# yassouali/pytorch-segmentation

Measured on NVIDIA H100. Metric: images/sec DeepLabV3+/ResNet101 513x513 train step (fwd+CE+bwd+SGD), higher is better.
Workload: dtype bf16

## Files before the change

### pytorch-segmentation_b200/csrc/seg_conv_tc.cu

```cuda
#include <cuda.h>
#include <mutex>
#include <stdlib.h>
#include "seg_common.cuh"
#include "seg_ptx.cuh"
#include "seg_sync.cuh"

namespace seg {
namespace tc {

using namespace ptx;

constexpr int BM = 128;
constexpr int BK = 64;
constexpr int A_BYTES = BM * 128;
constexpr int KIND_KK = 0, KIND_KM = 1;
constexpr int NTHREADS = 384;
constexpr int NCONS = 256;
constexpr int MAXT = 49;

constexpr int BAR_CONSUMERS = 1;
constexpr int BAR_ORDER = 2;
constexpr int BAR_WG = 4;

struct TcParams {
  CUtensorMap mapA;
  CUtensorMap mapB;
  int M;
  int Ncols;
  int taps;
  int kchunks;
  int stride;
  int lower_h, lower_w;
  int PQ, Q;
  int x_im2col;
  int brows_per_tap;
  short tap_wt[MAXT];
  short tap_oh[MAXT];
  short tap_ow[MAXT];
  void* out;
  long long ldo;
  int out_dtype;
  float beta;
  const float* bias;
  double* stats;
  int stat_rows;
  unsigned* stat_ticket;
  SyncDesc sync;
  int out_strided, out_H, out_W, osy, osx, opy, opx;
  int n_tiles, tiles;
  int kblocks_total, kblocks_per_split;
  float* dw;
  int dw_K, dw_C;
  float* ws;
};

__device__ __forceinline__ void row_to_coords(int m, int PQ, int Q, int stride, int lower_h, int lower_w, int& n, int& h,
                                              int& w) {
  n = m / PQ;
  int rem = m - n * PQ;
  int pp = rem / Q;
  int qq = rem - pp * Q;
  h = lower_h + pp * stride;
  w = lower_w + qq * stride;
}

template <int BN, int TA, int TB>
__device__ __forceinline__ void wgmma_tile(float* acc, uint64_t adesc, uint64_t bdesc, uint32_t accumulate) {
  if constexpr (BN == 64) wgmma_m64n64k16<TA, TB>(acc, adesc, bdesc, accumulate);
  else if constexpr (BN == 128) wgmma_m64n128k16<TA, TB>(acc, adesc, bdesc, accumulate);
  else wgmma_m64n256k16<TA, TB>(acc, adesc, bdesc, accumulate);
}

template <int BN, int KIND>
__device__ __forceinline__ void load_kblock(const TcParams& p, uint32_t a_dst, uint32_t bar, int kc, int wtap, uint16_t oh,
                                            uint16_t ow, int n_img, int h0, int w0, int m0, int n0) {
  const uint32_t b_dst = a_dst + A_BYTES;
  if (p.x_im2col)
    tma_load_im2col_4d(a_dst, &p.mapA, bar, kc * BK, w0, h0, n_img, ow, oh);
  else
    tma_load_2d(a_dst, &p.mapA, bar, kc * BK, m0);
  if (KIND == KIND_KK) {
    tma_load_2d(b_dst, &p.mapB, bar, kc * BK, wtap * p.brows_per_tap + n0);
  } else {
#pragma unroll
    for (int j = 0; j < BN / 64; ++j)
      tma_load_2d(b_dst + j * 8192, &p.mapB, bar, n0 + j * 64, wtap * p.brows_per_tap + kc * BK);
  }
}

template <int BN>
__device__ __forceinline__ void stage_acc(const float* acc, const float* acc1, uint8_t* stage, int rbase, int warp, int lane,
                                          const float* bias, bool out_f32) {
  const int esize = out_f32 ? 4 : 2;
  const int CPR = BN * esize / 16;
  const int swz = (CPR >= 32 ? 31 : CPR - 1);
  const int r0 = rbase + warp * 16 + (lane >> 2);
#pragma unroll
  for (int j = 0; j < BN / 8; ++j) {
    const int col = j * 8 + 2 * (lane & 3);
    float b0 = 0.f, b1 = 0.f;
    if (bias) {
      b0 = bias[col];
      b1 = bias[col + 1];
    }
#pragma unroll
    for (int h = 0; h < 4; ++h) {
      if (h >= 2 && !acc1) break;
      const float* a = h < 2 ? acc : acc1;
      const int r = r0 + 8 * (h & 1) + 32 * (h & 2);
      const float x0 = a[4 * j + 2 * (h & 1)] + b0, x1 = a[4 * j + 2 * (h & 1) + 1] + b1;
      const int byte = col * esize;
      uint8_t* dst = stage + (size_t)r * (BN * esize) + ((((byte >> 4) ^ (r & swz))) << 4) + (byte & 15);
      if (out_f32)
        *reinterpret_cast<float2*>(dst) = make_float2(x0, x1);
      else
        *reinterpret_cast<__nv_bfloat162*>(dst) = __floats2bfloat162_rn(x0, x1);
    }
  }
}


template <int BN, int ESIZE>
__device__ __forceinline__ void store_tile(const TcParams& p, const uint8_t* stage, int tid, int m0, int n0, int ncols_tile) {
  constexpr int CPR = BN * ESIZE / 16;
  constexpr int swz = (CPR >= 32 ? 31 : CPR - 1);
  constexpr int RSTEP = 128 / CPR;
  constexpr int NCH = BM / RSTEP;
  constexpr int BATCH = 8;
  static_assert(128 % CPR == 0 && NCH % BATCH == 0, "chunk walk of the staged tile");
  const int c16 = tid % CPR;
  const int nchunks = (ncols_tile * ESIZE + 15) >> 4;
  if (c16 >= nchunks) return;
  const bool vec_ok = ((p.ldo * ESIZE) & 15) == 0 && ((reinterpret_cast<uintptr_t>(p.out) + (size_t)n0 * ESIZE) & 15) == 0;
  const int first_col = (c16 << 4) / ESIZE;
  const bool full = first_col + 16 / ESIZE <= ncols_tile;
  auto row_dst = [&](int tr) {
    const int grow = m0 + tr;
    long long pixel = grow;
    if (p.out_strided) {
      const int n = grow / p.PQ;
      const int rem = grow - n * p.PQ;
      const int i = rem / p.Q, jj = rem - i * p.Q;
      pixel = ((long long)n * p.out_H + (i * p.osy + p.opy)) * p.out_W + (jj * p.osx + p.opx);
    }
    return reinterpret_cast<uint8_t*>(p.out) + ((size_t)pixel * p.ldo + n0) * ESIZE + ((size_t)c16 << 4);
  };
  auto row_src = [&](int tr) { return stage + (size_t)tr * (BN * ESIZE) + ((c16 ^ (tr & swz)) << 4); };
  if (ESIZE == 2 && vec_ok && full && p.beta != 0.f) {
    for (int b = 0; b < NCH; b += BATCH) {
      uint8_t* dst[BATCH];
      uint4 old[BATCH];
#pragma unroll
      for (int u = 0; u < BATCH; ++u) {
        const int tr = tid / CPR + (b + u) * RSTEP;
        dst[u] = m0 + tr < p.M ? row_dst(tr) : nullptr;
        old[u] = dst[u] ? *reinterpret_cast<const uint4*>(dst[u]) : make_uint4(0u, 0u, 0u, 0u);
      }
#pragma unroll
      for (int u = 0; u < BATCH; ++u) {
        if (!dst[u]) continue;
        float a[8], o[8];
        unpack8(*reinterpret_cast<const bf16x8*>(row_src(tid / CPR + (b + u) * RSTEP)), a);
        unpack8(*reinterpret_cast<const bf16x8*>(&old[u]), o);
#pragma unroll
        for (int k = 0; k < 8; ++k) a[k] += p.beta * o[k];
        *reinterpret_cast<bf16x8*>(dst[u]) = pack8(a);
      }
    }
    return;
  }
  for (int tr = tid / CPR; tr < BM; tr += RSTEP) {
    if (m0 + tr >= p.M) break;
    const uint8_t* src = row_src(tr);
    uint8_t* dst = row_dst(tr);
    if (ESIZE == 2 && vec_ok && full) {
      *reinterpret_cast<bf16x8*>(dst) = *reinterpret_cast<const bf16x8*>(src);
    } else if (ESIZE == 2) {
      float a[8];
      unpack8(*reinterpret_cast<const bf16x8*>(src), a);
      __nv_bfloat16* d = reinterpret_cast<__nv_bfloat16*>(dst);
      for (int k = 0; k < 8; ++k)
        if (first_col + k < ncols_tile) {
          float o = a[k];
          if (p.beta != 0.f) o += p.beta * bf2f(d[k]);
          d[k] = f2bf(o);
        }
    } else {
      const float4 val = *reinterpret_cast<const float4*>(src);
      const float a[4] = {val.x, val.y, val.z, val.w};
      float* d = reinterpret_cast<float*>(dst);
      if (vec_ok && full && p.beta == 0.f) {
        *reinterpret_cast<float4*>(d) = val;
      } else {
        for (int k = 0; k < 4; ++k)
          if (first_col + k < ncols_tile) d[k] = (p.beta != 0.f) ? a[k] + p.beta * d[k] : a[k];
      }
    }
  }
}

template <int BN>
struct PPCfg {
  static_assert(BN == 64 || BN == 128, "ping-pong tile width");
  static constexpr int B_BYTES = BN * 128;
  static constexpr int STAGE_BYTES = A_BYTES + B_BYTES;
  static constexpr int STAGES = BN == 64 ? 6 : 4;
  static constexpr int RING = STAGES * STAGE_BYTES;
  static constexpr int STG_BYTES = BM * 256;
  static constexpr int MAXG = BM / 32;
  static constexpr int STAT_BYTES = MAXG * 2 * BN * 4 + BN * 4;
  static constexpr int SMEM = RING + 2 * (STG_BYTES + STAT_BYTES) + 1024  + 256 ;
  static_assert(16 * STAGES + 8 <= 256, "barrier area");
  static_assert(SMEM <= 227 * 1024, "shared memory per block");
};

template <int BN, int KIND>
__global__ void __launch_bounds__(NTHREADS, 1) conv_gemm_pp(const __grid_constant__ TcParams p) {
  using C = PPCfg<BN>;
  constexpr int STAGES = C::STAGES;
  extern __shared__ uint8_t smem_raw[];
  const uint32_t raw_addr = smem_u32(smem_raw);
  const uint32_t smem0 = (raw_addr + 1023u) & ~1023u;
  uint8_t* smem_gen = smem_raw + (smem0 - raw_addr);
  const uint32_t bar0 = smem0 + C::RING + 2 * (C::STG_BYTES + C::STAT_BYTES);
  auto full_bar = [&](int s) { return bar0 + 8u * s; };
  auto empty_bar = [&](int s) { return bar0 + 8u * (STAGES + s); };
  volatile int* flag_sm = reinterpret_cast<volatile int*>(smem_gen + (bar0 - smem0) + 16 * STAGES);

  const int num_iters = p.taps * p.kchunks;
  const int grid = gridDim.x;
  const int ntiles = (p.tiles - (int)blockIdx.x + grid - 1) / grid;

  if (threadIdx.x == 0) {
    prefetch_tmap(&p.mapA);
    prefetch_tmap(&p.mapB);
    for (int s = 0; s < STAGES; ++s) {
      mbar_init(full_bar(s), 1);
      mbar_init(empty_bar(s), 4);
    }
    fence_mbar_init();
  }
  __syncthreads();
  pdl_wait();

  if (threadIdx.x < 128) {
    setmaxnreg_dec<40>();
    if (threadIdx.x == 0 && num_iters > 0) {
      int it = 0;
      for (int j = 0; j < ntiles; ++j) {
        const int t = blockIdx.x + j * grid;
        const int m0 = (t / p.n_tiles) * BM, n0 = (t % p.n_tiles) * BN;
        int n_img = 0, h0 = 0, w0 = 0;
        if (p.x_im2col) row_to_coords(m0, p.PQ, p.Q, p.stride, p.lower_h, p.lower_w, n_img, h0, w0);
        for (int tap = 0; tap < p.taps; ++tap) {
          const int wtap = p.tap_wt[tap];
          const uint16_t oh = (uint16_t)p.tap_oh[tap], ow = (uint16_t)p.tap_ow[tap];
          for (int kc = 0; kc < p.kchunks; ++kc, ++it) {
            const int st = it % STAGES;
            mbar_wait_nocall(empty_bar(st), ((it / STAGES) & 1) ^ 1u);
            mbar_arrive_expect_tx(full_bar(st), C::STAGE_BYTES);
            load_kblock<BN, KIND>(p, smem0 + st * C::STAGE_BYTES, full_bar(st), kc, wtap, oh, ow, n_img, h0, w0, m0, n0);
          }
        }
      }
    }
    return;
  }

  setmaxnreg_inc<232>();
  const int cw = (threadIdx.x - 128) >> 7;
  const int tid = threadIdx.x & 127;
  const int warp = tid >> 5, lane = tid & 31;
  uint8_t* stage = smem_gen + C::RING + cw * C::STG_BYTES;
  float* stat_sm = reinterpret_cast<float*>(smem_gen + C::RING + 2 * C::STG_BYTES + cw * C::STAT_BYTES);
  float* bias_sm = stat_sm + C::MAXG * 2 * BN;
  const bool out_f32 = p.out_dtype != SEG_DT_BF16;
  const int esize = out_f32 ? 4 : 2;
  const int CPR = BN * esize / 16;
  const int swz = (CPR >= 32 ? 31 : CPR - 1);
  auto wg_sync = [&] { named_sync(BAR_WG + cw, 128); };

  for (int j = cw; j < ntiles; j += 2) {
    const int t = blockIdx.x + j * grid;
    const int m0 = (t / p.n_tiles) * BM, n0 = (t % p.n_tiles) * BN;
    float acc0[BN / 2], acc1[BN / 2];
#pragma unroll
    for (int i = 0; i < BN / 2; ++i) acc0[i] = acc1[i] = 0.f;

    if (j > 0) named_sync(BAR_ORDER + cw, NCONS);
    {
      constexpr int TB = (KIND == KIND_KK) ? 0 : 1;
      const int it0 = j * num_iters;
      for (int i = 0; i < num_iters; ++i) {
        const int it = it0 + i;
        const int st = it % STAGES;
        mbar_wait_nocall(full_bar(st), (it / STAGES) & 1);
        const uint32_t a_addr = smem0 + st * C::STAGE_BYTES;
        const uint32_t b_addr = a_addr + A_BYTES;
        const uint64_t adesc0 = make_smem_desc_sw128(a_addr, 16, 1024);
        const uint64_t adesc1 = make_smem_desc_sw128(a_addr + 8192, 16, 1024);
        const uint64_t bdesc0 = make_smem_desc_sw128(b_addr, TB ? 8192 : 16, 1024);
        wgmma_fence();
#pragma unroll
        for (int k = 0; k < BK / 16; ++k) {
          const uint64_t bdesc = bdesc0 + (uint64_t)(TB ? (k * 2048 >> 4) : (k * 32 >> 4));
          wgmma_tile<BN, 0, TB>(acc0, adesc0 + (uint64_t)(k * 32 >> 4), bdesc, 1u);
          wgmma_tile<BN, 0, TB>(acc1, adesc1 + (uint64_t)(k * 32 >> 4), bdesc, 1u);
        }
        wgmma_commit();
        wgmma_wait<1>();
        __syncwarp();
        if (i > 0 && lane == 0) mbar_arrive(empty_bar((it - 1) % STAGES));
      }
      if (j + 1 < ntiles) named_arrive(BAR_ORDER + (cw ^ 1), NCONS);
      wgmma_wait<0>();
      __syncwarp();
      if (num_iters > 0 && lane == 0) mbar_arrive(empty_bar((it0 + num_iters - 1) % STAGES));
    }

    const int ncols_tile = min(BN, p.Ncols - n0);
    if (p.bias && tid < BN) bias_sm[tid] = tid < ncols_tile ? __ldg(p.bias + n0 + tid) : 0.f;
    wg_sync();
    stage_acc<BN>(acc0, acc1, stage, 0, warp, lane, p.bias ? bias_sm : nullptr, out_f32);
    wg_sync();

    const int ngroups = BM / p.stat_rows;
    if (p.stats) {
      const int parts = min(128 / BN, ngroups);
      const int rpp = BM / parts;
      const int c = tid % BN, part = tid / BN;
      const int rvalid = min(BM, p.M - m0);
      if (part < parts) {
        const int byte = c * esize;
        int g = part * rpp / p.stat_rows;
        auto load = [&](int r) {
          const uint8_t* src = stage + (size_t)r * (BN * esize) + ((((byte >> 4) ^ (r & swz))) << 4) + (byte & 15);
          return out_f32 ? *reinterpret_cast<const float*>(src) : bf2f(*reinterpret_cast<const __nv_bfloat16*>(src));
        };
        for (int rg = part * rpp; rg < (part + 1) * rpp; rg += p.stat_rows, ++g) {
          float s1 = 0.f, s2 = 0.f;
          const int rend = min(rg + p.stat_rows, rvalid);
          int r = rg;
          for (; r + 8 <= rend; r += 8) {
            float x[8];
#pragma unroll
            for (int u = 0; u < 8; ++u) x[u] = load(r + u);
#pragma unroll
            for (int u = 0; u < 8; ++u) {
              s1 += x[u];
              s2 = fmaf(x[u], x[u], s2);
            }
          }
          for (; r < rend; ++r) {
            const float x = load(r);
            s1 += x;
            s2 = fmaf(x, x, s2);
          }
          stat_sm[(g * 2 + 0) * BN + c] = s1;
          stat_sm[(g * 2 + 1) * BN + c] = s2;
        }
      }
    }

    if (out_f32)
      store_tile<BN, 4>(p, stage, tid, m0, n0, ncols_tile);
    else
      store_tile<BN, 2>(p, stage, tid, m0, n0, ncols_tile);
    if (j == ntiles - 1 && tid == 0) pdl_trigger();

    if (p.stats) {
      wg_sync();
      if (tid < ncols_tile) {
        float a = 0.f, b = 0.f;
        for (int g = 0; g < ngroups; ++g) {
          a += stat_sm[(g * 2 + 0) * BN + tid];
          b += stat_sm[(g * 2 + 1) * BN + tid];
        }
        atomicAdd(p.stats + n0 + tid, (double)a);
        atomicAdd(p.stats + p.Ncols + n0 + tid, (double)b);
      }
    }
  }

  if (p.stats && p.sync.world > 0)
    sync_push_when_last<false>(p.sync, p.stats, 2 * p.Ncols, p.stat_ticket, gridDim.x, threadIdx.x - 128, NCONS,
                               [] { named_sync(BAR_CONSUMERS, NCONS); }, flag_sm);
}


template <int BN>
struct Cfg {
  static constexpr int B_BYTES = BN * 128;
  static constexpr int STAGE_BYTES = A_BYTES + B_BYTES;
  static constexpr int STAGES = BN == 64 ? 6 : (BN == 128 ? 5 : 4);
  static constexpr int SMEM = STAGES * STAGE_BYTES + 1024  + 256 ;
  static_assert(STAGES * STAGE_BYTES >= BM * BN * 4, "staging tile must fit in the pipeline ring");
  static_assert(SMEM <= 227 * 1024, "shared memory per block");
};

template <int BN>
__global__ void __launch_bounds__(NTHREADS, 1) conv_gemm_wgrad(const __grid_constant__ TcParams p) {
  using C = Cfg<BN>;
  constexpr int STAGES = C::STAGES;
  extern __shared__ uint8_t smem_raw[];
  const uint32_t raw_addr = smem_u32(smem_raw);
  const uint32_t smem0 = (raw_addr + 1023u) & ~1023u;
  uint8_t* smem_gen = smem_raw + (smem0 - raw_addr);
  const uint32_t bar0 = smem0 + STAGES * C::STAGE_BYTES;
  auto full_bar = [&](int s) { return bar0 + 8u * s; };
  auto empty_bar = [&](int s) { return bar0 + 8u * (STAGES + s); };

  const int m0 = blockIdx.x * BM;
  const int n0 = blockIdx.y * BN;

  const int tap_mm = blockIdx.z % p.taps;
  const int split = blockIdx.z / p.taps;
  const int kb_begin = split * p.kblocks_per_split;
  const int kb_end = min(kb_begin + p.kblocks_per_split, p.kblocks_total);
  const int num_iters = max(kb_end - kb_begin, 0);

  if (threadIdx.x == 0) {
    prefetch_tmap(&p.mapA);
    prefetch_tmap(&p.mapB);
    for (int s = 0; s < STAGES; ++s) {
      mbar_init(full_bar(s), 1);
      mbar_init(empty_bar(s), 8);
    }
    fence_mbar_init();
  }
  __syncthreads();
  pdl_wait();

  if (threadIdx.x < 128) {
    if (threadIdx.x == 0 && num_iters > 0) {
      const uint16_t oh = (uint16_t)p.tap_oh[tap_mm], ow = (uint16_t)p.tap_ow[tap_mm];
      int it = 0;
      for (int kb = kb_begin; kb < kb_end; ++kb, ++it) {
        const int st = it % STAGES;
        const uint32_t ph = (it / STAGES) & 1;
        mbar_wait_nocall(empty_bar(st), ph ^ 1u);
        const uint32_t a_dst = smem0 + st * C::STAGE_BYTES;
        const uint32_t b_dst = a_dst + A_BYTES;
        const int pix0 = kb * BK;
        mbar_arrive_expect_tx(full_bar(st), C::STAGE_BYTES);
        tma_load_2d(a_dst, &p.mapA, full_bar(st), m0, pix0);
        tma_load_2d(a_dst + 8192, &p.mapA, full_bar(st), m0 + 64, pix0);
        if (p.x_im2col) {
          int n_img, h0, w0;
          row_to_coords(pix0, p.PQ, p.Q, p.stride, p.lower_h, p.lower_w, n_img, h0, w0);
#pragma unroll
          for (int j = 0; j < BN / 64; ++j)
            tma_load_im2col_4d(b_dst + j * 8192, &p.mapB, full_bar(st), n0 + j * 64, w0, h0, n_img, ow, oh);
        } else {
#pragma unroll
          for (int j = 0; j < BN / 64; ++j) tma_load_2d(b_dst + j * 8192, &p.mapB, full_bar(st), n0 + j * 64, pix0);
        }
      }
    }
    return;
  }

  if (num_iters == 0) return;
  const int ctid = threadIdx.x - 128;
  const int cw = ctid >> 7;
  const int warp = (ctid >> 5) & 3, lane = ctid & 31;
  float acc[BN / 2];
#pragma unroll
  for (int i = 0; i < BN / 2; ++i) acc[i] = 0.f;
  for (int it = 0; it < num_iters; ++it) {
    const int st = it % STAGES;
    mbar_wait_nocall(full_bar(st), (it / STAGES) & 1);
    const uint32_t a_addr = smem0 + st * C::STAGE_BYTES + cw * 8192;
    const uint32_t b_addr = smem0 + st * C::STAGE_BYTES + A_BYTES;
    const uint64_t adesc0 = make_smem_desc_sw128(a_addr, 8192, 1024);
    const uint64_t bdesc0 = make_smem_desc_sw128(b_addr, 8192, 1024);
    wgmma_fence();
#pragma unroll
    for (int k = 0; k < BK / 16; ++k)
      wgmma_tile<BN, 1, 1>(acc, adesc0 + (uint64_t)(k * 2048 >> 4), bdesc0 + (uint64_t)(k * 2048 >> 4), 1u);
    wgmma_commit();
    wgmma_wait<1>();
    __syncwarp();
    if (it > 0 && lane == 0) mbar_arrive(empty_bar((it - 1) % STAGES));
  }
  wgmma_wait<0>();
  named_sync(BAR_CONSUMERS, NCONS);

  uint8_t* stage = smem_gen;
  const int ncols_tile = min(BN, p.Ncols - n0);
  stage_acc<BN>(acc, nullptr, stage, cw * 64, warp, lane, nullptr, true);
  named_sync(BAR_CONSUMERS, NCONS);

  const int CPR = BN * 4 / 16;
  const int swz = (CPR >= 32 ? 31 : CPR - 1);
  float* base = p.ws ? p.ws + (size_t)split * p.taps * p.dw_K * p.dw_C : p.dw;
  for (int idx = ctid; idx < BM * CPR; idx += NCONS) {
    const int tr = idx / CPR, c16 = idx - tr * CPR;
    const int row = m0 + tr, col0 = c16 * 4;
    if (row >= p.M || col0 >= ncols_tile) continue;
    const float4 v = *reinterpret_cast<const float4*>(stage + (size_t)tr * (BN * 4) + ((c16 ^ (tr & swz)) << 4));
    float* dst = base + ((size_t)tap_mm * p.dw_K + row) * p.dw_C + n0 + col0;
    const bool vec = col0 + 4 <= ncols_tile && ((reinterpret_cast<uintptr_t>(dst) & 15) == 0);
    const float a[4] = {v.x, v.y, v.z, v.w};
    if (p.ws) {
      if (vec)
        *reinterpret_cast<float4*>(dst) = v;
      else
        for (int i = 0; i < 4; ++i)
          if (col0 + i < ncols_tile) dst[i] = a[i];
    } else if (vec) {
      asm volatile("red.global.add.v4.f32 [%0], {%1, %2, %3, %4};" ::"l"(dst), "f"(v.x), "f"(v.y), "f"(v.z), "f"(v.w)
                   : "memory");
    } else {
      for (int i = 0; i < 4; ++i)
        if (col0 + i < ncols_tile) atomicAdd(dst + i, a[i]);
    }
  }
}

typedef CUresult (*EncodeTiledFn)(CUtensorMap*, CUtensorMapDataType, cuuint32_t, void*, const cuuint64_t*,
                                  const cuuint64_t*, const cuuint32_t*, const cuuint32_t*, CUtensorMapInterleave,
                                  CUtensorMapSwizzle, CUtensorMapL2promotion, CUtensorMapFloatOOBfill);
typedef CUresult (*EncodeIm2colFn)(CUtensorMap*, CUtensorMapDataType, cuuint32_t, void*, const cuuint64_t*,
                                   const cuuint64_t*, const int*, const int*, cuuint32_t, cuuint32_t,
                                   const cuuint32_t*, CUtensorMapInterleave, CUtensorMapSwizzle,
                                   CUtensorMapL2promotion, CUtensorMapFloatOOBfill);
static EncodeTiledFn g_encode_tiled = nullptr;
static EncodeIm2colFn g_encode_im2col = nullptr;
static int g_driver_version = 0;

static int resolve_driver() {
  static std::once_flag once;
  static int status = 0;
  std::call_once(once, [] {
    void* f1 = nullptr;
    void* f2 = nullptr;
    cudaDriverEntryPointQueryResult q;
    if (cudaGetDriverEntryPoint("cuTensorMapEncodeTiled", &f1, cudaEnableDefault, &q) != cudaSuccess || !f1) status = 1;
    if (cudaGetDriverEntryPoint("cuTensorMapEncodeIm2col", &f2, cudaEnableDefault, &q) != cudaSuccess || !f2) status = 1;
    g_encode_tiled = (EncodeTiledFn)f1;
    g_encode_im2col = (EncodeIm2colFn)f2;
    cudaDriverGetVersion(&g_driver_version);
  });
  if (status) set_error("cannot resolve cuTensorMapEncode* driver entry points");
  return status;
}

static int make_map_2d(CUtensorMap* m, const void* ptr, int64_t rows, int64_t cols, int64_t ld, int box_rows) {
  if (resolve_driver()) return 1;
  SEG_REQUIRE((reinterpret_cast<uintptr_t>(ptr) & 15) == 0, "TMA: base pointer not 16-byte aligned");
  SEG_REQUIRE(ld % 8 == 0, "TMA: row pitch %lld not a multiple of 8 elements", (long long)ld);
  cuuint64_t dims[2] = {(cuuint64_t)cols, (cuuint64_t)rows};
  cuuint64_t strides[1] = {(cuuint64_t)ld * 2};
  cuuint32_t box[2] = {64, (cuuint32_t)box_rows};
  cuuint32_t es[2] = {1, 1};
  CUresult r = g_encode_tiled(m, CU_TENSOR_MAP_DATA_TYPE_BFLOAT16, 2, const_cast<void*>(ptr), dims, strides, box, es,
                              CU_TENSOR_MAP_INTERLEAVE_NONE, CU_TENSOR_MAP_SWIZZLE_128B,
                              CU_TENSOR_MAP_L2_PROMOTION_L2_256B, CU_TENSOR_MAP_FLOAT_OOB_FILL_NONE);
  SEG_REQUIRE(r == CUDA_SUCCESS, "cuTensorMapEncodeTiled failed (%d) rows=%lld cols=%lld ld=%lld box_rows=%d", (int)r,
              (long long)rows, (long long)cols, (long long)ld, box_rows);
  return 0;
}

static int make_map_im2col(CUtensorMap* m, const void* ptr, int N, int H, int W, int C, int64_t ld, int lower_w,
                           int lower_h, int upper_w, int upper_h, int stride, int pixels) {
  if (resolve_driver()) return 1;
  SEG_REQUIRE((reinterpret_cast<uintptr_t>(ptr) & 15) == 0, "TMA: base pointer not 16-byte aligned");
  SEG_REQUIRE(ld % 8 == 0, "TMA: channel pitch %lld not a multiple of 8", (long long)ld);
  SEG_REQUIRE(lower_w >= -128 && upper_w >= -128 && lower_w <= 127 && upper_w <= 127 && lower_h >= -128 &&
                  upper_h >= -128 && lower_h <= 127 && upper_h <= 127,
              "im2col corner out of range");
  cuuint64_t dims[4] = {(cuuint64_t)C, (cuuint64_t)W, (cuuint64_t)H, (cuuint64_t)N};
  cuuint64_t strides[3] = {(cuuint64_t)ld * 2, (cuuint64_t)W * ld * 2, (cuuint64_t)H * W * ld * 2};
  int lo[2] = {lower_w, lower_h};
  int up[2] = {upper_w, upper_h};
  cuuint32_t es[4] = {1, (cuuint32_t)stride, (cuuint32_t)stride, 1};
  CUresult r = g_encode_im2col(m, CU_TENSOR_MAP_DATA_TYPE_BFLOAT16, 4, const_cast<void*>(ptr), dims, strides, lo, up,
                               64, (cuuint32_t)pixels, es, CU_TENSOR_MAP_INTERLEAVE_NONE, CU_TENSOR_MAP_SWIZZLE_128B,
                               CU_TENSOR_MAP_L2_PROMOTION_L2_256B, CU_TENSOR_MAP_FLOAT_OOB_FILL_NONE);
  SEG_REQUIRE(r == CUDA_SUCCESS,
              "cuTensorMapEncodeIm2col failed (%d) N=%d H=%d W=%d C=%d ld=%lld lo=(%d,%d) up=(%d,%d) s=%d", (int)r, N, H,
              W, C, (long long)ld, lower_w, lower_h, upper_w, upper_h, stride);
  if (g_driver_version <= 13010) {
    const uint64_t bytes = (uint64_t)N * H * W * ld * 2;
    if (bytes < 131072) reinterpret_cast<uint64_t*>(m)[1] &= ~(1ull << 21);
  }
  return 0;
}

template <int BN, int KIND>
static int launch_pp(TcParams& p, cudaStream_t stream) {
  static bool attr_set = false;
  auto kfn = conv_gemm_pp<BN, KIND>;
  if (!attr_set) {
    cudaError_t e = cudaFuncSetAttribute(kfn, cudaFuncAttributeMaxDynamicSharedMemorySize, PPCfg<BN>::SMEM);
    SEG_REQUIRE(e == cudaSuccess, "cudaFuncSetAttribute(smem=%d): %s", PPCfg<BN>::SMEM, cudaGetErrorString(e));
    attr_set = true;
  }
  const int n_tiles = ceil_div(p.Ncols, BN);
  const int64_t tiles = ceil_div64(p.M, BM) * n_tiles;
  SEG_REQUIRE(tiles < (1ll << 31), "too many output tiles");
  p.n_tiles = n_tiles;
  p.tiles = (int)tiles;
  const dim3 grid((unsigned)std::min<int64_t>(tiles, num_sms()));
  launch_pdl(kfn, grid, dim3(NTHREADS), (size_t)PPCfg<BN>::SMEM, stream, p);
  return check_launch("conv_gemm_pp");
}

template <int KIND>
static int launch_pp_bn(int bn, TcParams& p, cudaStream_t stream) {
  switch (bn) {
    case 64: return launch_pp<64, KIND>(p, stream);
    case 128: return launch_pp<128, KIND>(p, stream);
  }
  set_error("bad BN %d", bn);
  return 1;
}

template <int BN>
static int launch_wgrad(const TcParams& p, dim3 grid, cudaStream_t stream) {
  static bool attr_set = false;
  auto kfn = conv_gemm_wgrad<BN>;
  if (!attr_set) {
    cudaError_t e = cudaFuncSetAttribute(kfn, cudaFuncAttributeMaxDynamicSharedMemorySize, Cfg<BN>::SMEM);
    SEG_REQUIRE(e == cudaSuccess, "cudaFuncSetAttribute(smem=%d): %s", Cfg<BN>::SMEM, cudaGetErrorString(e));
    attr_set = true;
  }
  launch_pdl(kfn, grid, dim3(NTHREADS), (size_t)Cfg<BN>::SMEM, stream, p);
  return check_launch("conv_gemm_wgrad");
}

static int launch_wgrad_bn(int bn, const TcParams& p, dim3 grid, cudaStream_t stream) {
  switch (bn) {
    case 64: return launch_wgrad<64>(p, grid, stream);
    case 128: return launch_wgrad<128>(p, grid, stream);
    case 256: return launch_wgrad<256>(p, grid, stream);
  }
  set_error("bad BN %d", bn);
  return 1;
}

static int pick_bn(int ncols, bool out_f32) { return (ncols <= 64 || out_f32) ? 64 : 128; }

static int stat_rows_for(int ncols) {
  if (ncols <= 64) return 32;
  if (ncols < 256) return 64;
  return ceil_div(ncols, 256) * 256 - ncols < 128 ? 128 : 64;
}

bool supported(const seg_conv_desc* d) {
  if (d->C % 8 != 0 || d->ldx % 8 != 0) return false;
  if (d->R != d->S) return false;
  if (d->R * d->S > MAXT) return false;
  if (d->pad > 127 || d->dil * (d->R - 1) - d->pad > 127 || d->dil * (d->R - 1) - d->pad < -127) return false;
  if (d->stride > 8) return false;
  return true;
}

static bool is_pointwise(const seg_conv_desc* d) { return d->R == 1 && d->S == 1 && d->stride == 1 && d->pad == 0; }

int conv_fwd(const seg_conv_desc* d, const void* x, const void* w, void* y, int y_dtype, const float* bias, float beta,
             double* stats, unsigned* stat_ticket, const SyncDesc* sync, cudaStream_t stream) {
  SEG_REQUIRE(supported(d), "wgmma conv fwd: unsupported shape (C=%d ldx=%d R=%d pad=%d dil=%d)", d->C, d->ldx, d->R,
              d->pad, d->dil);
  TcParams p;
  memset(&p, 0, sizeof(p));
  const int64_t M = (int64_t)d->N * d->P * d->Q;
  SEG_REQUIRE(M < (1ll << 31), "M too large");
  p.M = (int)M;
  p.Ncols = d->K;
  p.taps = d->R * d->S;
  for (int t = 0; t < p.taps; ++t) {
    p.tap_wt[t] = (short)t;
    p.tap_oh[t] = (short)((t / d->S) * d->dil);
    p.tap_ow[t] = (short)((t % d->S) * d->dil);
  }
  p.kchunks = ceil_div(d->C, BK);
  p.stride = d->stride;
  p.lower_h = p.lower_w = -d->pad;
  p.PQ = d->P * d->Q;
  p.Q = d->Q;
  p.brows_per_tap = d->K;
  p.out = y;
  p.ldo = d->ldy;
  p.out_dtype = y_dtype;
  p.beta = beta;
  p.bias = bias;
  p.stats = stats;
  p.stat_ticket = stat_ticket;
  if (sync && stats) {
    SEG_REQUIRE(stat_ticket != nullptr, "conv fwd: SyncBN needs a zeroed ticket word");
    SEG_REQUIRE(4 * d->K <= sync->n_max, "conv fwd: 2*K = %d fp64 statistics exceed the SyncBN buffer (%d floats)", 2 * d->K, sync->n_max);
    p.sync = *sync;
  }
  const int bn = pick_bn(d->K, y_dtype != SEG_DT_BF16);
  p.stat_rows = stat_rows_for(d->K);
  if (is_pointwise(d)) {
    p.x_im2col = 0;
    if (make_map_2d(&p.mapA, x, M, d->C, d->ldx, BM)) return 1;
  } else {
    p.x_im2col = 1;
    const int upper = d->pad - (d->R - 1) * d->dil;
    if (make_map_im2col(&p.mapA, x, d->N, d->H, d->W, d->C, d->ldx, -d->pad, -d->pad, upper, upper, d->stride, BM)) return 1;
  }
  if (make_map_2d(&p.mapB, w, (int64_t)p.taps * d->K, d->C, d->C, bn)) return 1;
  return launch_pp_bn<KIND_KK>(bn, p, stream);
}

static int floordiv(int a, int b) { return (a >= 0) ? a / b : -((-a + b - 1) / b); }

int conv_dgrad(const seg_conv_desc* d, const void* dy, const void* w, void* dx, float beta, cudaStream_t stream) {
  SEG_REQUIRE(supported(d) && d->ldy % 8 == 0, "wgmma conv dgrad: unsupported shape (stride=%d K=%d ldy=%d)", d->stride,
              d->K, d->ldy);
  const int s = d->stride;
  const int bn = pick_bn(d->C, false);
  for (int py = 0; py < s; ++py) {
    for (int px = 0; px < s; ++px) {
      const int Hs = (d->H - py + s - 1) / s, Ws = (d->W - px + s - 1) / s;
      if (Hs <= 0 || Ws <= 0) continue;
      TcParams p;
      memset(&p, 0, sizeof(p));
      int rh[8], oh[8], nh = 0, rw[8], ow[8], nw = 0;
      for (int r = 0; r < d->R; ++r) {
        const int num = py + d->pad - r * d->dil;
        if (((num % s) + s) % s == 0) { rh[nh] = r; oh[nh] = floordiv(num, s); ++nh; }
      }
      for (int q = 0; q < d->S; ++q) {
        const int num = px + d->pad - q * d->dil;
        if (((num % s) + s) % s == 0) { rw[nw] = q; ow[nw] = floordiv(num, s); ++nw; }
      }
      int min_oh = 0, min_ow = 0;
      for (int i = 0; i < nh; ++i) min_oh = (i == 0) ? oh[i] : min(min_oh, oh[i]);
      for (int i = 0; i < nw; ++i) min_ow = (i == 0) ? ow[i] : min(min_ow, ow[i]);
      p.taps = nh * nw;
      for (int i = 0; i < nh; ++i)
        for (int j = 0; j < nw; ++j) {
          const int t = i * nw + j;
          p.tap_wt[t] = (short)(rh[i] * d->S + rw[j]);
          p.tap_oh[t] = (short)(oh[i] - min_oh);
          p.tap_ow[t] = (short)(ow[j] - min_ow);
        }
      const int64_t M = (int64_t)d->N * Hs * Ws;
      SEG_REQUIRE(M < (1ll << 31), "M too large");
      p.M = (int)M;
      p.Ncols = d->C;
      p.kchunks = ceil_div(d->K, BK);
      p.stride = 1;
      p.lower_h = min_oh;
      p.lower_w = min_ow;
      p.PQ = Hs * Ws;
      p.Q = Ws;
      p.brows_per_tap = d->K;
      p.out = dx;
      p.ldo = d->ldx;
      p.out_dtype = SEG_DT_BF16;
      p.beta = beta;
      if (s > 1) {
        p.out_strided = 1;
        p.out_H = d->H;
        p.out_W = d->W;
        p.osy = p.osx = s;
        p.opy = py;
        p.opx = px;
      }
      p.stat_rows = BM;
      if (p.taps > 0) {
        const bool plain = (s == 1 && is_pointwise(d));
        if (plain) {
          p.x_im2col = 0;
          if (make_map_2d(&p.mapA, dy, M, d->K, d->ldy, BM)) return 1;
        } else {
          p.x_im2col = 1;
          const int upper_h = Hs - d->P + min_oh, upper_w = Ws - d->Q + min_ow;
          if (make_map_im2col(&p.mapA, dy, d->N, d->P, d->Q, d->K, d->ldy, min_ow, min_oh, upper_w, upper_h, 1, BM)) return 1;
        }
        if (make_map_2d(&p.mapB, w, (int64_t)d->R * d->S * d->K, d->C, d->C, 64)) return 1;
      } else {
        if (beta == 1.f) continue;
        if (make_map_2d(&p.mapA, w, (int64_t)d->R * d->S * d->K, d->C, d->C, BM)) return 1;
        if (make_map_2d(&p.mapB, w, (int64_t)d->R * d->S * d->K, d->C, d->C, 64)) return 1;
      }
      if (launch_pp_bn<KIND_KM>(bn, p, stream)) return 1;
    }
  }
  return 0;
}

__global__ void wgrad_split_reduce_kernel(const float* __restrict__ ws, int splits, int64_t n, float* __restrict__ dw) {
  for (int64_t i = blockIdx.x * (int64_t)blockDim.x + threadIdx.x; i < n; i += (int64_t)gridDim.x * blockDim.x) {
    float acc = ws[i];
    for (int s = 1; s < splits; ++s) acc += ws[(size_t)s * n + i];
    dw[i] += acc;
  }
}

static void wgrad_plan(const seg_conv_desc* d, int& bn, int& splits, int& kblocks_per_split) {
  const bool wide = d->R * d->S >= 9 && d->C >= 256 && d->C % 256 == 0;
  bn = (d->C <= 64) ? 64 : (wide ? 256 : 128);
  const int kblocks_total = (int)ceil_div64((int64_t)d->N * d->P * d->Q, BK);
  const int tiles = ceil_div(d->K, BM) * ceil_div(d->C, bn) * d->R * d->S;
  splits = max(1, num_sms() / tiles);
  splits = min(splits, kblocks_total);
  splits = min(splits, 1024);
  kblocks_per_split = ceil_div(kblocks_total, splits);
  splits = ceil_div(kblocks_total, kblocks_per_split);
}

int64_t wgrad_workspace_floats(const seg_conv_desc* d) {
  if (!supported(d)) return 0;
  int bn, splits, kps;
  wgrad_plan(d, bn, splits, kps);
  return splits > 1 ? (int64_t)splits * d->R * d->S * d->K * d->C : 0;
}

int conv_wgrad(const seg_conv_desc* d, const void* dy, const void* x, float* dw, float* ws, cudaStream_t stream) {
  SEG_REQUIRE(supported(d) && d->ldy % 8 == 0, "wgmma conv wgrad: unsupported shape");
  TcParams p;
  memset(&p, 0, sizeof(p));
  const int64_t npix = (int64_t)d->N * d->P * d->Q;
  SEG_REQUIRE(npix < (1ll << 31), "too many pixels");
  p.M = d->K;
  p.Ncols = d->C;
  p.taps = d->R * d->S;
  for (int t = 0; t < p.taps; ++t) {
    p.tap_wt[t] = (short)t;
    p.tap_oh[t] = (short)((t / d->S) * d->dil);
    p.tap_ow[t] = (short)((t % d->S) * d->dil);
  }
  p.stride = d->stride;
  p.lower_h = p.lower_w = -d->pad;
  p.PQ = d->P * d->Q;
  p.Q = d->Q;
  p.dw = dw;
  p.dw_K = d->K;
  p.dw_C = d->C;
  p.kblocks_total = (int)ceil_div64(npix, BK);
  int bn, splits;
  wgrad_plan(d, bn, splits, p.kblocks_per_split);
  SEG_REQUIRE(splits == 1 || ws != nullptr, "wgmma conv wgrad: %d k-splits need the workspace (seg_conv2d_wgrad_workspace_floats)", splits);
  SEG_REQUIRE((int64_t)(splits - 1) * p.kblocks_per_split < p.kblocks_total, "wgmma conv wgrad: split %d has no k-blocks", splits - 1);
  if (splits > 1) p.ws = ws;
  if (make_map_2d(&p.mapA, dy, npix, d->K, d->ldy, 64)) return 1;
  if (is_pointwise(d)) {
    p.x_im2col = 0;
    if (make_map_2d(&p.mapB, x, npix, d->C, d->ldx, 64)) return 1;
  } else {
    p.x_im2col = 1;
    const int upper = d->pad - (d->R - 1) * d->dil;
    if (make_map_im2col(&p.mapB, x, d->N, d->H, d->W, d->C, d->ldx, -d->pad, -d->pad, upper, upper, d->stride, 64)) return 1;
  }
  SEG_REQUIRE((unsigned)(p.taps * splits) <= 65535u, "wgrad grid.z too large");
  dim3 grid((unsigned)ceil_div(d->K, BM), (unsigned)ceil_div(d->C, bn), (unsigned)(p.taps * splits));
  if (launch_wgrad_bn(bn, p, grid, stream)) return 1;
  if (splits == 1) return 0;
  const int64_t n = (int64_t)p.taps * d->K * d->C;
  wgrad_split_reduce_kernel<<<(unsigned)std::min<int64_t>(ceil_div64(n, 256), (int64_t)num_sms() * 8), 256, 0, stream>>>(ws, splits, n, dw);
  return check_launch("wgrad_split_reduce");
}

}
}
```

### pytorch-segmentation_b200/csrc/seg_ptx.cuh

```cuda
#pragma once
#include <cuda.h>
#include <stdint.h>

namespace seg {
namespace ptx {

__device__ __forceinline__ uint32_t smem_u32(const void* p) { return (uint32_t)__cvta_generic_to_shared(p); }

__device__ __forceinline__ void mbar_init(uint32_t bar, uint32_t count) {
  asm volatile("mbarrier.init.shared::cta.b64 [%0], %1;" ::"r"(bar), "r"(count) : "memory");
}
__device__ __forceinline__ void fence_mbar_init() {
  asm volatile("fence.mbarrier_init.release.cluster;" ::: "memory");
}
__device__ __forceinline__ void fence_proxy_async() {
  asm volatile("fence.proxy.async.shared::cta;" ::: "memory");
}
__device__ __forceinline__ void mbar_arrive(uint32_t bar) {
  asm volatile("mbarrier.arrive.shared::cta.b64 _, [%0];" ::"r"(bar) : "memory");
}
__device__ __forceinline__ void mbar_arrive_expect_tx(uint32_t bar, uint32_t bytes) {
  asm volatile("mbarrier.arrive.expect_tx.shared::cta.b64 _, [%0], %1;" ::"r"(bar), "r"(bytes) : "memory");
}
__device__ __forceinline__ uint32_t mbar_try_wait(uint32_t bar, uint32_t parity) {
  uint32_t ok;
  asm volatile(
      "{\n\t.reg .pred p;\n\t"
      "mbarrier.try_wait.parity.shared::cta.b64 p, [%1], %2;\n\t"
      "selp.u32 %0, 1, 0, p;\n\t}"
      : "=r"(ok)
      : "r"(bar), "r"(parity)
      : "memory");
  return ok;
}
__device__ __forceinline__ void mbar_wait(uint32_t bar, uint32_t parity) {
  if (mbar_try_wait(bar, parity)) return;
  long long t0 = clock64();
  while (!mbar_try_wait(bar, parity)) {
    if (clock64() - t0 > 4000000000ll) {
      printf("seg_b200: mbarrier wait timeout (block %d,%d,%d thread %d bar %u parity %u)\n", blockIdx.x,
             blockIdx.y, blockIdx.z, threadIdx.x, bar, parity);
      __trap();
    }
  }
}

__device__ __forceinline__ void mbar_wait_nocall(uint32_t bar, uint32_t parity) {
  if (mbar_try_wait(bar, parity)) return;
  long long t0 = clock64();
  while (!mbar_try_wait(bar, parity))
    if (clock64() - t0 > 4000000000ll) __trap();
}

__device__ __forceinline__ void prefetch_tmap(const CUtensorMap* m) {
  asm volatile("prefetch.tensormap [%0];" ::"l"(reinterpret_cast<uint64_t>(m)) : "memory");
}
__device__ __forceinline__ void tma_load_2d(uint32_t dst, const CUtensorMap* m, uint32_t bar, int c0, int c1) {
  asm volatile(
      "cp.async.bulk.tensor.2d.shared::cluster.global.mbarrier::complete_tx::bytes [%0], [%1, {%3, %4}], [%2];" ::"r"(dst),
      "l"(reinterpret_cast<uint64_t>(m)), "r"(bar), "r"(c0), "r"(c1)
      : "memory");
}
__device__ __forceinline__ void tma_load_im2col_4d(uint32_t dst, const CUtensorMap* m, uint32_t bar, int c, int w,
                                                   int h, int n, uint16_t off_w, uint16_t off_h) {
  asm volatile(
      "cp.async.bulk.tensor.4d.shared::cluster.global.im2col.mbarrier::complete_tx::bytes [%0], [%1, {%3, %4, %5, "
      "%6}], [%2], {%7, %8};" ::"r"(dst),
      "l"(reinterpret_cast<uint64_t>(m)), "r"(bar), "r"(c), "r"(w), "r"(h), "r"(n), "h"(off_w), "h"(off_h)
      : "memory");
}

template <int N>
__device__ __forceinline__ void setmaxnreg_inc() { asm volatile("setmaxnreg.inc.sync.aligned.u32 %0;" ::"n"(N)); }
template <int N>
__device__ __forceinline__ void setmaxnreg_dec() { asm volatile("setmaxnreg.dec.sync.aligned.u32 %0;" ::"n"(N)); }
__device__ __forceinline__ void named_sync(int id, int count) {
  asm volatile("bar.sync %0, %1;" ::"r"(id), "r"(count) : "memory");
}
__device__ __forceinline__ void named_arrive(int id, int count) {
  asm volatile("bar.arrive %0, %1;" ::"r"(id), "r"(count) : "memory");
}

__device__ __forceinline__ void wgmma_fence() { asm volatile("wgmma.fence.sync.aligned;" ::: "memory"); }
__device__ __forceinline__ void wgmma_commit() { asm volatile("wgmma.commit_group.sync.aligned;" ::: "memory"); }
template <int N>
__device__ __forceinline__ void wgmma_wait() { asm volatile("wgmma.wait_group.sync.aligned %0;" ::"n"(N) : "memory"); }

__device__ __forceinline__ uint64_t make_smem_desc_sw128(uint32_t smem_addr, uint32_t lbo_bytes, uint32_t sbo_bytes) {
  uint64_t d = 0;
  d |= (uint64_t)((smem_addr & 0x3FFFFu) >> 4);
  d |= (uint64_t)((lbo_bytes >> 4) & 0x3FFFu) << 16;
  d |= (uint64_t)((sbo_bytes >> 4) & 0x3FFFu) << 32;
  d |= (uint64_t)1 << 62;
  return d;
}

template <int TA, int TB>
__device__ __forceinline__ void wgmma_m64n64k16(float* d, uint64_t adesc, uint64_t bdesc, uint32_t accumulate) {
  asm volatile(
      "{\n\t.reg .pred p;\n\tsetp.ne.b32 p, %34, 0;\n\t"
      "wgmma.mma_async.sync.aligned.m64n64k16.f32.bf16.bf16 "
      "{%0, %1, %2, %3, %4, %5, %6, %7, %8, %9, %10, %11, %12, %13, %14, %15, %16, %17, %18, %19, %20, %21, %22, %23, %24, %25, %26, %27, %28, %29, %30, %31}, %32, %33, p, 1, 1, %35, %36;\n\t}"
      : "+f"(d[0]), "+f"(d[1]), "+f"(d[2]), "+f"(d[3]), "+f"(d[4]), "+f"(d[5]), "+f"(d[6]), "+f"(d[7]), "+f"(d[8]), "+f"(d[9]), "+f"(d[10]), "+f"(d[11]), "+f"(d[12]), "+f"(d[13]), "+f"(d[14]), "+f"(d[15]), "+f"(d[16]), "+f"(d[17]), "+f"(d[18]), "+f"(d[19]), "+f"(d[20]), "+f"(d[21]), "+f"(d[22]), "+f"(d[23]), "+f"(d[24]), "+f"(d[25]), "+f"(d[26]), "+f"(d[27]), "+f"(d[28]), "+f"(d[29]), "+f"(d[30]), "+f"(d[31])
      : "l"(adesc), "l"(bdesc), "r"(accumulate), "n"(TA), "n"(TB)
      : "memory");
}

template <int TA, int TB>
__device__ __forceinline__ void wgmma_m64n128k16(float* d, uint64_t adesc, uint64_t bdesc, uint32_t accumulate) {
  asm volatile(
      "{\n\t.reg .pred p;\n\tsetp.ne.b32 p, %66, 0;\n\t"
      "wgmma.mma_async.sync.aligned.m64n128k16.f32.bf16.bf16 "
      "{%0, %1, %2, %3, %4, %5, %6, %7, %8, %9, %10, %11, %12, %13, %14, %15, %16, %17, %18, %19, %20, %21, %22, %23, %24, %25, %26, %27, %28, %29, %30, %31, %32, %33, %34, %35, %36, %37, %38, %39, %40, %41, %42, %43, %44, %45, %46, %47, %48, %49, %50, %51, %52, %53, %54, %55, %56, %57, %58, %59, %60, %61, %62, %63}, %64, %65, p, 1, 1, %67, %68;\n\t}"
      : "+f"(d[0]), "+f"(d[1]), "+f"(d[2]), "+f"(d[3]), "+f"(d[4]), "+f"(d[5]), "+f"(d[6]), "+f"(d[7]), "+f"(d[8]), "+f"(d[9]), "+f"(d[10]), "+f"(d[11]), "+f"(d[12]), "+f"(d[13]), "+f"(d[14]), "+f"(d[15]), "+f"(d[16]), "+f"(d[17]), "+f"(d[18]), "+f"(d[19]), "+f"(d[20]), "+f"(d[21]), "+f"(d[22]), "+f"(d[23]), "+f"(d[24]), "+f"(d[25]), "+f"(d[26]), "+f"(d[27]), "+f"(d[28]), "+f"(d[29]), "+f"(d[30]), "+f"(d[31]), "+f"(d[32]), "+f"(d[33]), "+f"(d[34]), "+f"(d[35]), "+f"(d[36]), "+f"(d[37]), "+f"(d[38]), "+f"(d[39]), "+f"(d[40]), "+f"(d[41]), "+f"(d[42]), "+f"(d[43]), "+f"(d[44]), "+f"(d[45]), "+f"(d[46]), "+f"(d[47]), "+f"(d[48]), "+f"(d[49]), "+f"(d[50]), "+f"(d[51]), "+f"(d[52]), "+f"(d[53]), "+f"(d[54]), "+f"(d[55]), "+f"(d[56]), "+f"(d[57]), "+f"(d[58]), "+f"(d[59]), "+f"(d[60]), "+f"(d[61]), "+f"(d[62]), "+f"(d[63])
      : "l"(adesc), "l"(bdesc), "r"(accumulate), "n"(TA), "n"(TB)
      : "memory");
}

template <int TA, int TB>
__device__ __forceinline__ void wgmma_m64n256k16(float* d, uint64_t adesc, uint64_t bdesc, uint32_t accumulate) {
  asm volatile(
      "{\n\t.reg .pred p;\n\tsetp.ne.b32 p, %130, 0;\n\t"
      "wgmma.mma_async.sync.aligned.m64n256k16.f32.bf16.bf16 "
      "{%0, %1, %2, %3, %4, %5, %6, %7, %8, %9, %10, %11, %12, %13, %14, %15, %16, %17, %18, %19, %20, %21, %22, %23, %24, %25, %26, %27, %28, %29, %30, %31, %32, %33, %34, %35, %36, %37, %38, %39, %40, %41, %42, %43, %44, %45, %46, %47, %48, %49, %50, %51, %52, %53, %54, %55, %56, %57, %58, %59, %60, %61, %62, %63, %64, %65, %66, %67, %68, %69, %70, %71, %72, %73, %74, %75, %76, %77, %78, %79, %80, %81, %82, %83, %84, %85, %86, %87, %88, %89, %90, %91, %92, %93, %94, %95, %96, %97, %98, %99, %100, %101, %102, %103, %104, %105, %106, %107, %108, %109, %110, %111, %112, %113, %114, %115, %116, %117, %118, %119, %120, %121, %122, %123, %124, %125, %126, %127}, %128, %129, p, 1, 1, %131, %132;\n\t}"
      : "+f"(d[0]), "+f"(d[1]), "+f"(d[2]), "+f"(d[3]), "+f"(d[4]), "+f"(d[5]), "+f"(d[6]), "+f"(d[7]), "+f"(d[8]), "+f"(d[9]), "+f"(d[10]), "+f"(d[11]), "+f"(d[12]), "+f"(d[13]), "+f"(d[14]), "+f"(d[15]), "+f"(d[16]), "+f"(d[17]), "+f"(d[18]), "+f"(d[19]), "+f"(d[20]), "+f"(d[21]), "+f"(d[22]), "+f"(d[23]), "+f"(d[24]), "+f"(d[25]), "+f"(d[26]), "+f"(d[27]), "+f"(d[28]), "+f"(d[29]), "+f"(d[30]), "+f"(d[31]), "+f"(d[32]), "+f"(d[33]), "+f"(d[34]), "+f"(d[35]), "+f"(d[36]), "+f"(d[37]), "+f"(d[38]), "+f"(d[39]), "+f"(d[40]), "+f"(d[41]), "+f"(d[42]), "+f"(d[43]), "+f"(d[44]), "+f"(d[45]), "+f"(d[46]), "+f"(d[47]), "+f"(d[48]), "+f"(d[49]), "+f"(d[50]), "+f"(d[51]), "+f"(d[52]), "+f"(d[53]), "+f"(d[54]), "+f"(d[55]), "+f"(d[56]), "+f"(d[57]), "+f"(d[58]), "+f"(d[59]), "+f"(d[60]), "+f"(d[61]), "+f"(d[62]), "+f"(d[63]), "+f"(d[64]), "+f"(d[65]), "+f"(d[66]), "+f"(d[67]), "+f"(d[68]), "+f"(d[69]), "+f"(d[70]), "+f"(d[71]), "+f"(d[72]), "+f"(d[73]), "+f"(d[74]), "+f"(d[75]), "+f"(d[76]), "+f"(d[77]), "+f"(d[78]), "+f"(d[79]), "+f"(d[80]), "+f"(d[81]), "+f"(d[82]), "+f"(d[83]), "+f"(d[84]), "+f"(d[85]), "+f"(d[86]), "+f"(d[87]), "+f"(d[88]), "+f"(d[89]), "+f"(d[90]), "+f"(d[91]), "+f"(d[92]), "+f"(d[93]), "+f"(d[94]), "+f"(d[95]), "+f"(d[96]), "+f"(d[97]), "+f"(d[98]), "+f"(d[99]), "+f"(d[100]), "+f"(d[101]), "+f"(d[102]), "+f"(d[103]), "+f"(d[104]), "+f"(d[105]), "+f"(d[106]), "+f"(d[107]), "+f"(d[108]), "+f"(d[109]), "+f"(d[110]), "+f"(d[111]), "+f"(d[112]), "+f"(d[113]), "+f"(d[114]), "+f"(d[115]), "+f"(d[116]), "+f"(d[117]), "+f"(d[118]), "+f"(d[119]), "+f"(d[120]), "+f"(d[121]), "+f"(d[122]), "+f"(d[123]), "+f"(d[124]), "+f"(d[125]), "+f"(d[126]), "+f"(d[127])
      : "l"(adesc), "l"(bdesc), "r"(accumulate), "n"(TA), "n"(TB)
      : "memory");
}

}
}
```

Measured before the change: 373.0.

## Store bf16 conv epilogue via stmatrix staging and TMA bulk tensor stores

Adds a TMA store path for bf16 conv outputs. Accumulators are written to shared memory in 64-column, 128B-swizzled slabs using stmatrix, then one thread issues cp.async.bulk.tensor stores, or reduce-add stores when beta=1. This replaces the per-thread vectorized global store loop and frees the consumer warps sooner, with bulk-group waits guarding reuse of the staging buffer. The BN statistics fold is adapted to read the new staging layout. It is on by default through an environment flag and falls back for unaligned, strided or f32 outputs.

Measured after the change: 382.6 (median of 6 runs). 1.03x the previous value.

```diff
diff --git a/pytorch-segmentation_b200/csrc/seg_conv_tc.cu b/pytorch-segmentation_b200/csrc/seg_conv_tc.cu
--- a/pytorch-segmentation_b200/csrc/seg_conv_tc.cu
+++ b/pytorch-segmentation_b200/csrc/seg_conv_tc.cu
@@ -1,5 +1,6 @@
 #include <cuda.h>
 #include <mutex>
+#include <type_traits>
 #include <stdlib.h>
 #include "seg_common.cuh"
 #include "seg_ptx.cuh"
@@ -22,9 +23,15 @@
 constexpr int BAR_ORDER = 2;
 constexpr int BAR_WG = 4;
 
+constexpr int STORE_THREADS = 0;
+constexpr int STORE_TMA = 1;
+constexpr int STORE_TMA_ADD = 2;
+
 struct TcParams {
   CUtensorMap mapA;
   CUtensorMap mapB;
+  CUtensorMap mapO;
+  int store_mode;
   int M;
   int Ncols;
   int taps;
@@ -119,6 +126,39 @@
   }
 }
 
+__device__ __forceinline__ int stg_tma(int r, int c16) { return (c16 >> 3) * (BM * 128) + r * 128 + (((c16 & 7) ^ (r & 7)) << 4); }
+
+template <int BN>
+__device__ __forceinline__ void stage_acc_tma(const float* acc0, const float* acc1, uint8_t* stage, int warp, int lane,
+                                              const float* bias) {
+  const int mi = lane >> 3;
+  const int col = 2 * (lane & 3);
+  const uint32_t stage_s = smem_u32(stage);
+#pragma unroll
+  for (int h = 0; h < 2; ++h) {
+    const float* a = h == 0 ? acc0 : acc1;
+    const int r = 64 * h + warp * 16 + (mi & 1) * 8 + (lane & 7);
+#pragma unroll
+    for (int jj = 0; jj < BN / 16; ++jj) {
+      float b0 = 0.f, b1 = 0.f, b2 = 0.f, b3 = 0.f;
+      if (bias) {
+        b0 = bias[16 * jj + col];
+        b1 = bias[16 * jj + col + 1];
+        b2 = bias[16 * jj + 8 + col];
+        b3 = bias[16 * jj + 8 + col + 1];
+      }
+      uint32_t v[4];
+#pragma unroll
+      for (int i = 0; i < 4; ++i) {
+        const __nv_bfloat162 x = __floats2bfloat162_rn(a[8 * jj + 2 * i] + (i < 2 ? b0 : b2),
+                                                       a[8 * jj + 2 * i + 1] + (i < 2 ? b1 : b3));
+        v[i] = *reinterpret_cast<const uint32_t*>(&x);
+      }
+      stmatrix_x4(stage_s + stg_tma(r, 2 * jj + (mi >> 1)), v[0], v[1], v[2], v[3]);
+    }
+  }
+}
+
 
 template <int BN, int ESIZE>
 __device__ __forceinline__ void store_tile(const TcParams& p, const uint8_t* stage, int tid, int m0, int n0, int ncols_tile) {
@@ -234,6 +274,7 @@
   if (threadIdx.x == 0) {
     prefetch_tmap(&p.mapA);
     prefetch_tmap(&p.mapB);
+    if (p.store_mode != STORE_THREADS) prefetch_tmap(&p.mapO);
     for (int s = 0; s < STAGES; ++s) {
       mbar_init(full_bar(s), 1);
       mbar_init(empty_bar(s), 4);
@@ -278,6 +319,7 @@
   const int esize = out_f32 ? 4 : 2;
   const int CPR = BN * esize / 16;
   const int swz = (CPR >= 32 ? 31 : CPR - 1);
+  const bool tma_store = p.store_mode != STORE_THREADS;
   auto wg_sync = [&] { named_sync(BAR_WG + cw, 128); };
 
   for (int j = cw; j < ntiles; j += 2) {
@@ -320,9 +362,27 @@
 
     const int ncols_tile = min(BN, p.Ncols - n0);
     if (p.bias && tid < BN) bias_sm[tid] = tid < ncols_tile ? __ldg(p.bias + n0 + tid) : 0.f;
+    if (tma_store && tid == 0) bulk_wait_all<true>();
     wg_sync();
-    stage_acc<BN>(acc0, acc1, stage, 0, warp, lane, p.bias ? bias_sm : nullptr, out_f32);
+    if (tma_store) {
+      stage_acc_tma<BN>(acc0, acc1, stage, warp, lane, p.bias ? bias_sm : nullptr);
+      fence_proxy_async();
+    } else {
+      stage_acc<BN>(acc0, acc1, stage, 0, warp, lane, p.bias ? bias_sm : nullptr, out_f32);
+    }
     wg_sync();
+
+    if (tma_store && tid == 0) {
+#pragma unroll
+      for (int b = 0; b < BN / 64; ++b) {
+        if (b * 64 >= ncols_tile) break;
+        if (p.store_mode == STORE_TMA_ADD)
+          tma_store_2d<true>(&p.mapO, smem_u32(stage) + b * (BM * 128), n0 + b * 64, m0);
+        else
+          tma_store_2d<false>(&p.mapO, smem_u32(stage) + b * (BM * 128), n0 + b * 64, m0);
+      }
+      bulk_commit();
+    }
 
     const int ngroups = BM / p.stat_rows;
     if (p.stats) {
@@ -332,41 +392,54 @@
       const int rvalid = min(BM, p.M - m0);
       if (part < parts) {
         const int byte = c * esize;
-        int g = part * rpp / p.stat_rows;
-        auto load = [&](int r) {
-          const uint8_t* src = stage + (size_t)r * (BN * esize) + ((((byte >> 4) ^ (r & swz))) << 4) + (byte & 15);
-          return out_f32 ? *reinterpret_cast<const float*>(src) : bf2f(*reinterpret_cast<const __nv_bfloat16*>(src));
+        auto fold = [&](auto tma_layout) {
+          int g = part * rpp / p.stat_rows;
+          auto load = [&](int r) {
+            if constexpr (decltype(tma_layout)::value)
+              return bf2f(*reinterpret_cast<const __nv_bfloat16*>(stage + stg_tma(r, byte >> 4) + (byte & 15)));
+            else {
+              const uint8_t* src = stage + (size_t)r * (BN * esize) + ((((byte >> 4) ^ (r & swz))) << 4) + (byte & 15);
+              return out_f32 ? *reinterpret_cast<const float*>(src) : bf2f(*reinterpret_cast<const __nv_bfloat16*>(src));
+            }
+          };
+          for (int rg = part * rpp; rg < (part + 1) * rpp; rg += p.stat_rows, ++g) {
+            float s1 = 0.f, s2 = 0.f;
+            const int rend = min(rg + p.stat_rows, rvalid);
+            int r = rg;
+            for (; r + 8 <= rend; r += 8) {
+              float x[8];
+#pragma unroll
+              for (int u = 0; u < 8; ++u) x[u] = load(r + u);
+#pragma unroll
+              for (int u = 0; u < 8; ++u) {
+                s1 += x[u];
+                s2 = fmaf(x[u], x[u], s2);
+              }
+            }
+            for (; r < rend; ++r) {
+              const float x = load(r);
+              s1 += x;
+              s2 = fmaf(x, x, s2);
+            }
+            stat_sm[(g * 2 + 0) * BN + c] = s1;
+            stat_sm[(g * 2 + 1) * BN + c] = s2;
+          }
         };
-        for (int rg = part * rpp; rg < (part + 1) * rpp; rg += p.stat_rows, ++g) {
-          float s1 = 0.f, s2 = 0.f;
-          const int rend = min(rg + p.stat_rows, rvalid);
-          int r = rg;
-          for (; r + 8 <= rend; r += 8) {
-            float x[8];
-#pragma unroll
-            for (int u = 0; u < 8; ++u) x[u] = load(r + u);
-#pragma unroll
-            for (int u = 0; u < 8; ++u) {
-              s1 += x[u];
-              s2 = fmaf(x[u], x[u], s2);
-            }
-          }
-          for (; r < rend; ++r) {
-            const float x = load(r);
-            s1 += x;
-            s2 = fmaf(x, x, s2);
-          }
-          stat_sm[(g * 2 + 0) * BN + c] = s1;
-          stat_sm[(g * 2 + 1) * BN + c] = s2;
-        }
+        if (tma_store)
+          fold(std::true_type{});
+        else
+          fold(std::false_type{});
       }
     }
 
     if (out_f32)
       store_tile<BN, 4>(p, stage, tid, m0, n0, ncols_tile);
-    else
+    else if (!tma_store)
       store_tile<BN, 2>(p, stage, tid, m0, n0, ncols_tile);
-    if (j == ntiles - 1 && tid == 0) pdl_trigger();
+    if (j == ntiles - 1 && tid == 0) {
+      if (tma_store) bulk_wait_all<false>();
+      pdl_trigger();
+    }
 
     if (p.stats) {
       wg_sync();
@@ -381,6 +454,7 @@
       }
     }
   }
+  if (tma_store && tid == 0) bulk_wait_all<false>();
 
   if (p.stats && p.sync.world > 0)
     sync_push_when_last<false>(p.sync, p.stats, 2 * p.Ncols, p.stat_ticket, gridDim.x, threadIdx.x - 128, NCONS,
@@ -588,6 +662,25 @@
   return 0;
 }
 
+static bool tma_store_enabled() {
+  static int v = -1;
+  if (v < 0) {
+    const char* e = getenv("SEG_CONV_TMA_STORE");
+    v = e ? atoi(e) : 1;
+  }
+  return v != 0;
+}
+
+static int pick_store_mode(TcParams& p) {
+  p.store_mode = STORE_THREADS;
+  if (!tma_store_enabled() || p.out_dtype != SEG_DT_BF16 || p.out_strided || p.M <= 0) return 0;
+  if (p.beta != 0.f && p.beta != 1.f) return 0;
+  if ((reinterpret_cast<uintptr_t>(p.out) & 15) != 0 || p.ldo % 8 != 0 || p.ldo < p.Ncols || p.ldo >= (1ll << 39)) return 0;
+  if (make_map_2d(&p.mapO, p.out, p.M, p.Ncols, p.ldo, BM)) return 1;
+  p.store_mode = p.beta == 0.f ? STORE_TMA : STORE_TMA_ADD;
+  return 0;
+}
+
 template <int BN, int KIND>
 static int launch_pp(TcParams& p, cudaStream_t stream) {
   static bool attr_set = false;
@@ -704,6 +797,7 @@
     if (make_map_im2col(&p.mapA, x, d->N, d->H, d->W, d->C, d->ldx, -d->pad, -d->pad, upper, upper, d->stride, BM)) return 1;
   }
   if (make_map_2d(&p.mapB, w, (int64_t)p.taps * d->K, d->C, d->C, bn)) return 1;
+  if (pick_store_mode(p)) return 1;
   return launch_pp_bn<KIND_KK>(bn, p, stream);
 }
 
@@ -780,6 +874,7 @@
         if (make_map_2d(&p.mapA, w, (int64_t)d->R * d->S * d->K, d->C, d->C, BM)) return 1;
         if (make_map_2d(&p.mapB, w, (int64_t)d->R * d->S * d->K, d->C, d->C, 64)) return 1;
       }
+      if (pick_store_mode(p)) return 1;
       if (launch_pp_bn<KIND_KM>(bn, p, stream)) return 1;
     }
   }
diff --git a/pytorch-segmentation_b200/csrc/seg_ptx.cuh b/pytorch-segmentation_b200/csrc/seg_ptx.cuh
--- a/pytorch-segmentation_b200/csrc/seg_ptx.cuh
+++ b/pytorch-segmentation_b200/csrc/seg_ptx.cuh
@@ -70,6 +70,29 @@
       : "memory");
 }
 
+template <bool REDUCE>
+__device__ __forceinline__ void tma_store_2d(const CUtensorMap* m, uint32_t src, int c0, int c1) {
+  if constexpr (REDUCE)
+    asm volatile("cp.reduce.async.bulk.tensor.2d.global.shared::cta.add.tile.bulk_group [%0, {%2, %3}], [%1];" ::"l"(
+                     reinterpret_cast<uint64_t>(m)), "r"(src), "r"(c0), "r"(c1)
+                 : "memory");
+  else
+    asm volatile("cp.async.bulk.tensor.2d.global.shared::cta.tile.bulk_group [%0, {%2, %3}], [%1];" ::"l"(
+                     reinterpret_cast<uint64_t>(m)), "r"(src), "r"(c0), "r"(c1)
+                 : "memory");
+}
+__device__ __forceinline__ void bulk_commit() { asm volatile("cp.async.bulk.commit_group;" ::: "memory"); }
+template <bool READ>
+__device__ __forceinline__ void bulk_wait_all() {
+  if constexpr (READ) asm volatile("cp.async.bulk.wait_group.read 0;" ::: "memory");
+  else asm volatile("cp.async.bulk.wait_group 0;" ::: "memory");
+}
+__device__ __forceinline__ void stmatrix_x4(uint32_t addr, uint32_t r0, uint32_t r1, uint32_t r2, uint32_t r3) {
+  asm volatile("stmatrix.sync.aligned.m8n8.x4.shared.b16 [%0], {%1, %2, %3, %4};" ::"r"(addr), "r"(r0), "r"(r1), "r"(r2),
+               "r"(r3)
+               : "memory");
+}
+
 template <int N>
 __device__ __forceinline__ void setmaxnreg_inc() { asm volatile("setmaxnreg.inc.sync.aligned.u32 %0;" ::"n"(N)); }
 template <int N>
```
